# h33p/ofps

Hardware: AMD Instinct MI355X
Metric: Mvectors/s, 1080p 16x16 blocks +-16 full-search SAD (higher is better)
Workload: dtype u8

## Files before the change

### ofps_amd/csrc/sad.hip

```cpp
#include "common.hpp"

#include <cstdlib>
#include <utility>

namespace {

constexpr int kWavesPerWG = 4;

constexpr int pick_stride(int min_s, int k, int ng) {
    for (int s = min_s; s < min_s + 64; ++s)
        if ((k * s) % 32 == ng % 32) return s;
    return min_s | 1;
}

template <int B, int R, int K>
struct SadCfg {
    static_assert(B % 4 == 0 && R % 4 == 0, "tile origin must stay dword aligned");
    static_assert(B * B * 255 <= 65535, "packed u16 SAD accumulators would overflow");
    static constexpr int NCAND = 2 * R + 1;
    static constexpr int NG = (NCAND + 3) / 4;
    static constexpr int NC = (NCAND + K - 1) / K;
    static constexpr int T = NG * NC;
    static constexpr int PASSES = (T + 63) / 64;
    static constexpr int BW = B / 4;
    static constexpr int TILE_H = B + 2 * R;
    static constexpr int TILE_ROWS = NC * K + B - 1;
    static constexpr int TILE_WD = (kWavesPerWG * B + 2 * R) / 4;
    static constexpr int MAXCOL = (kWavesPerWG - 1) * BW + (NG - 1) + BW;
    static constexpr int MIN_S = (MAXCOL + 1 > TILE_WD) ? MAXCOL + 1 : TILE_WD;
    static constexpr int S = pick_stride(MIN_S, K, NG);
    static constexpr int LDS_DWORDS = TILE_ROWS * S;
};

__device__ __forceinline__ unsigned long long shfl_xor_u64(unsigned long long v, int mask) {
    unsigned lo = (unsigned)v, hi = (unsigned)(v >> 32);
    lo = __shfl_xor(lo, mask, 64);
    hi = __shfl_xor(hi, mask, 64);
    return ((unsigned long long)hi << 32) | lo;
}

struct __attribute__((packed, aligned(4))) U64A4 { unsigned long long v; };

struct SadParams {
    const uint8_t* prev_base;
    const uint8_t* cur_base;
    size_t prev_pitch, cur_pitch;
    int W, H, stride;
    int nbx, nby;
    float nx, ny;
    float4* out_entries;
    int* out_best;
    unsigned long long div_spp, div_spr;
};
inline unsigned long long div_magic48(unsigned d) { return ((1ull << 48) + d - 1) / d; }
__device__ __forceinline__ unsigned div48(unsigned n, unsigned long long m) { return (unsigned)(((unsigned long long)n * m) >> 48); }

__device__ __forceinline__ void write_block_result(const SadParams& p, int pair, int bx, int by, int B, int R,
                                                   unsigned long long key) {
    const int sad = (int)(key >> 48);
    const int dy = (int)((key >> 8) & 0xFF) - R;
    const int dx = (int)(key & 0xFF) - R;
    const size_t k = ((size_t)pair * p.nby + by) * p.nbx + bx;
    const float cx = (float)(bx * B + B / 2 + dx), cy = (float)(by * B + B / 2 + dy);
    float4 e;
    e.x = cx * p.nx;
    e.y = cy * p.ny;
    e.z = ((float)dx / 1.0f) * (-p.nx);
    e.w = ((float)dy / 1.0f) * (-p.ny);
    p.out_entries[k] = e;
    if (p.out_best) {
        p.out_best[3 * k + 0] = dx;
        p.out_best[3 * k + 1] = dy;
        p.out_best[3 * k + 2] = sad;
    }
}

template <int B, int R, int K>
__global__ __launch_bounds__(256) void sad_qsad_kernel(const SadParams p) {
    using C = SadCfg<B, R, K>;
    __shared__ uint32_t tile[C::LDS_DWORDS];

    const int pair = blockIdx.z;
    const uint8_t* __restrict__ prev = p.prev_base + (size_t)pair * p.prev_pitch;
    const uint8_t* __restrict__ cur = p.cur_base + (size_t)pair * p.cur_pitch;
    const int by = blockIdx.y;
    const int bx0 = blockIdx.x * kWavesPerWG;
    const int tid = threadIdx.x;

    const int wave = __builtin_amdgcn_readfirstlane(tid >> 6);
    const int lane = tid & 63;
    const int bx = bx0 + wave;
    const int x0 = bx * B, y0 = by * B;

    uint32_t c[B][C::BW];
    {
        const int bxc = bx < p.nbx ? bx : p.nbx - 1;
        const uint32_t* __restrict__ cp = reinterpret_cast<const uint32_t*>(cur + (size_t)y0 * p.stride + bxc * B);
        const int sdw = p.stride >> 2;
#pragma unroll
        for (int y = 0; y < B; ++y)
#pragma unroll
            for (int q = 0; q < C::BW; ++q) c[y][q] = cp[y * sdw + q];
    }

    {
        const int tx0 = bx0 * B - R, ty0 = by * B - R;
        for (int idx = tid; idx < C::TILE_H * C::TILE_WD; idx += 256) {
            const int row = idx / C::TILE_WD, col = idx - row * C::TILE_WD;
            const int gx = tx0 + 4 * col, gy = ty0 + row;
            if (gy >= 0 && gy < p.H && gx >= 0 && gx < p.W)
                tile[row * C::S + col] = *reinterpret_cast<const uint32_t*>(prev + (size_t)gy * p.stride + gx);
        }
    }
    __syncthreads();
    if (bx >= p.nbx) return;

    unsigned long long best = ~0ull;
#pragma unroll 1
    for (int pass = 0; pass < C::PASSES; ++pass) {
        const int t = pass * 64 + lane;
        const bool active = t < C::T;
        const int tc = active ? t : 0;
        const int chunk = tc / C::NG, g = tc - chunk * C::NG;
        const int dx0 = -R + 4 * g, dy0 = -R + K * chunk;

        unsigned long long acc[K];
#pragma unroll
        for (int i = 0; i < K; ++i) acc[i] = 0;

        const uint32_t* trow = tile + (K * chunk) * C::S + wave * C::BW + g;
#pragma unroll
        for (int rr = 0; rr < B + K - 1; ++rr) {
            unsigned long long win[C::BW];
#pragma unroll
            for (int q = 0; q < C::BW; ++q) win[q] = reinterpret_cast<const U64A4*>(trow + rr * C::S + q)->v;
#pragma unroll
            for (int i = 0; i < K; ++i) {
                const int y = rr - i;
                if (y >= 0 && y < B) {
#pragma unroll
                    for (int q = 0; q < C::BW; ++q) acc[i] = __builtin_amdgcn_qsad_pk_u16_u8(win[q], c[y][q], acc[i]);
                }
            }
        }
        __builtin_amdgcn_sched_group_barrier(0x100, C::BW, 0);
#pragma unroll
        for (int rr = 0; rr < B + K - 1; ++rr) {
            __builtin_amdgcn_sched_group_barrier(0x100, C::BW, 0);
            __builtin_amdgcn_sched_group_barrier(0x002, K * C::BW, 0);
        }

#pragma unroll
        for (int i = 0; i < K; ++i) asm volatile("" : "+v"(acc[i]));

        uint32_t bkey = 0xFFFFFFFFu;
        int bci = 0;
#pragma unroll
        for (int i = 0; i < K; ++i) {
            const int dy = dy0 + i;
            const int vy = (int)active & (int)(dy <= R) & (int)(y0 + dy >= 0) & (int)(y0 + dy + B <= p.H);
#pragma unroll
            for (int j = 0; j < 4; ++j) {
                const int dx = dx0 + j;
                const int v = vy & (int)(dx <= R) & (int)(x0 + dx >= 0) & (int)(x0 + dx + B <= p.W);
                const uint32_t d2inv = (uint32_t)(dx * dx + dy * dy) | (uint32_t)(v - 1);
                const uint32_t half = (j < 2) ? (uint32_t)acc[i] : (uint32_t)(acc[i] >> 32);
                const uint32_t key = ((j & 1) ? (half & 0xFFFF0000u) : (half << 16)) | d2inv;
                const bool lt = key < bkey;
                bkey = lt ? key : bkey;
                bci = lt ? (i * 4 + j) : bci;
            }
        }
        if (bkey != 0xFFFFFFFFu) {
            const int bi = bci >> 2, bj = bci & 3;
            const unsigned long long k64 =
                ((unsigned long long)bkey << 32) | (uint32_t)(((dy0 + bi + R) << 8) | (dx0 + bj + R));
            best = k64 < best ? k64 : best;
        }
    }

#pragma unroll
    for (int m = 32; m >= 1; m >>= 1) {
        const unsigned long long o = shfl_xor_u64(best, m);
        best = o < best ? o : best;
    }
    if (lane == 0) write_block_result(p, pair, bx, by, B, R, best);
}

template <int B, int R>
struct StripCfg {
    static_assert(B % 4 == 0 && R % 4 == 0, "tile origin and the dx = +R column must stay dword aligned");
    static_assert(B * B * 255 <= 65535, "packed u16 SAD accumulators would overflow");
    static constexpr int NCAND = 2 * R + 1;
    static constexpr int NGA = (2 * R) / 4;
    static constexpr int pow2_ceil(int v) { int p = 1; while (p < v) p <<= 1; return p; }
    static constexpr int NG = pow2_ceil(NGA);
    static_assert(NGA >= 1 && NG <= 64, "search range too wide for one wave per strip");
    static constexpr int NB = 64 / NG;
    static constexpr int BW = B / 4;
    static constexpr int TILE_H = B + 2 * R;
    static constexpr int KE = (NCAND + NG - 1) / NG;
    static constexpr int EDGE_COL = (2 * R) / 4;
    static constexpr int GRAN = ((NB * B) % 16 == 0 && R % 16 == 0) ? 16 : (((NB * B) % 8 == 0 && R % 8 == 0) ? 8 : 4);
    static constexpr int GDW = GRAN / 4;
    static constexpr int TILE_WG = (NB * B + 2 * R + GRAN - 1) / GRAN;
    static constexpr int MAXCOL = (NB - 1) * BW + (NG - 1) + BW;
    static constexpr int SW = ((MAXCOL + 1 > TILE_WG * GDW ? MAXCOL + 1 : TILE_WG * GDW) + 3) / 4 * 4;
    static_assert((NB - 1) * BW + EDGE_COL + BW <= SW, "edge column must lie inside a window row");
    static constexpr int TILE_ROWS = TILE_H > NG * KE + B - 1 ? TILE_H : NG * KE + B - 1;
    static constexpr int TILE_DWORDS = TILE_ROWS * SW;
    static_assert(2 * R * R < 65536, "lane key holds d2 in 16 bits");
    static constexpr int SPLIT = (NCAND + 32) / 33;
    static constexpr int NP = (NCAND + SPLIT - 1) / SPLIT;
    static constexpr int MIN_WAVES = (2 * NP + B * BW + 40 <= 168) ? 3 : 2;
    static constexpr bool COMPACT_KEY = ((2 * R * R) << 6) + NCAND < 65536 && NCAND <= 64;
    static constexpr bool RANK_KEY = !COMPACT_KEY && ((2 * R * R) << 3) + 7 < 65536;
    static constexpr int KSHIFT = COMPACT_KEY ? 6 : (RANK_KEY ? 3 : 0);
};

template <int B, int R>
struct StripWalk {
    static constexpr int ROWS_PER_BASE = (255 - StripCfg<B, R>::BW) / StripCfg<B, R>::SW + 1;
};

template <int B, int R, int I0, int RR>
__device__ __forceinline__ void strip_row(unsigned long long (&acc)[StripCfg<B, R>::NP], const uint32_t (&c)[B][B / 4],
                                          const uint32_t* lds, uint32_t& base) {
    using C = StripCfg<B, R>;
    constexpr int G = StripWalk<B, R>::ROWS_PER_BASE;
    if constexpr (RR > 0 && RR % G == 0) {
        base += G * C::SW;
        asm volatile("" : "+v"(base));
    }
    unsigned long long win[C::BW];
#pragma unroll
    for (int q = 0; q < C::BW; ++q) win[q] = reinterpret_cast<const U64A4*>(lds + base + (RR % G) * C::SW + q)->v;
#pragma unroll
    for (int ii = 0; ii < C::NP; ++ii) {
        const int y = RR - ii;
        if (I0 + ii < C::NCAND && y >= 0 && y < B) {
#pragma unroll
            for (int q = 0; q < C::BW; ++q) acc[ii] = __builtin_amdgcn_qsad_pk_u16_u8(win[q], c[y][q], acc[ii]);
        }
    }
}

template <int B, int R, int I0, int... RR>
__device__ __forceinline__ void strip_rows(unsigned long long (&acc)[StripCfg<B, R>::NP], const uint32_t (&c)[B][B / 4],
                                           const uint32_t* lds, uint32_t tile_off, std::integer_sequence<int, RR...>) {
    uint32_t base = tile_off + I0 * StripCfg<B, R>::SW;
    asm volatile("" : "+v"(base));
    (strip_row<B, R, I0, RR>(acc, c, lds, base), ...);
}

#ifndef OFPS_SAD_COLKEYS
#define OFPS_SAD_COLKEYS 2
#endif
constexpr int kSadColKeys = OFPS_SAD_COLKEYS;
constexpr int kColSlotDwords = kSadColKeys == 2 ? 4 * 64 : 0;

template <int B, int R, int I0>
__device__ __forceinline__ void strip_pass(const uint32_t (&c)[B][B / 4], const uint32_t* lds, uint32_t tile_off,
                                           const uint32_t (&colk)[4], const uint32_t (&colk_pos)[4], int y0, int H, uint32_t& bkey, int& bi,
                                           uint32_t (&colmin)[4], uint32_t* amin) {
    using C = StripCfg<B, R>;
    unsigned long long acc[C::NP];
#pragma unroll
    for (int ii = 0; ii < C::NP; ++ii) acc[ii] = 0;
    constexpr int ROWS = ((I0 + C::NP < C::NCAND ? C::NP : C::NCAND - I0) + B - 1);
    strip_rows<B, R, I0>(acc, c, lds, tile_off, std::make_integer_sequence<int, ROWS>{});
#pragma unroll
    for (int ii = 0; ii < C::NP; ++ii) asm volatile("" : "+v"(acc[ii]));
    if constexpr (kSadColKeys != 0 && (C::RANK_KEY || C::COMPACT_KEY)) {
        auto low_of = [&](int ii) -> uint32_t {
            const int i = I0 + ii, dy = -R + i;
            const bool ok = i < C::NCAND && y0 + dy >= 0 && y0 + dy + B <= H;
            return ok ? (uint32_t)(C::RANK_KEY ? ((dy * dy) << 1 | (dy > 0 ? 1 : 0)) : ((dy * dy) << 6 | i)) : 0xFFFFFFFFu;
        };
        uint32_t hmask = 0xFFFF0000u;
        asm volatile("" : "+v"(hmask));
        auto keys_of = [&](int ii, uint32_t low, uint32_t (&k)[4]) {
            const uint32_t lo = (uint32_t)acc[ii], hi = (uint32_t)(acc[ii] >> 32);
            k[0] = (lo << 16) | low; k[1] = (lo & hmask) | low; k[2] = (hi << 16) | low; k[3] = (hi & hmask) | low;
        };
        if constexpr (kSadColKeys == 1) {
#pragma unroll
            for (int ii = 0; ii < C::NP; ii += 2) {
                if (I0 + ii >= C::NCAND) break;
                uint32_t ka[4], kb[4];
                keys_of(ii, low_of(ii), ka);
                if (ii + 1 < C::NP && I0 + ii + 1 < C::NCAND) {
                    keys_of(ii + 1, low_of(ii + 1), kb);
#pragma unroll
                    for (int j = 0; j < 4; ++j)
                        asm("v_min3_u32 %0, %1, %2, %3" : "=v"(colmin[j]) : "v"(colmin[j]), "v"(ka[j]), "v"(kb[j]));
                } else {
#pragma unroll
                    for (int j = 0; j < 4; ++j) colmin[j] = min(colmin[j], ka[j]);
                }
            }
        } else {
#pragma unroll
            for (int ii = 0; ii < C::NP; ++ii) {
                if (I0 + ii >= C::NCAND) break;
                uint32_t k[4];
                keys_of(ii, low_of(ii), k);
#pragma unroll
                for (int j = 0; j < 4; ++j) __hip_atomic_fetch_min(amin + 64 * j, k[j], __ATOMIC_RELAXED, __HIP_MEMORY_SCOPE_WAVEFRONT);
            }
        }
        return;
    }
#pragma unroll
    for (int ii = 0; ii < C::NP; ++ii) {
        const int i = I0 + ii;
        const int dy = -R + i;
        if (i < C::NCAND && y0 + dy >= 0 && y0 + dy + B <= H) {
            const uint32_t lo = (uint32_t)acc[ii], hi = (uint32_t)(acc[ii] >> 32);
            const uint32_t (&ck)[4] = (C::RANK_KEY && dy > 0) ? colk_pos : colk;
            const uint32_t k0 = (lo << 16) | ck[0];
            const uint32_t k1 = (lo & 0xFFFF0000u) | ck[1];
            const uint32_t k2 = (hi << 16) | ck[2];
            const uint32_t k3 = (hi & 0xFFFF0000u) | ck[3];
            if constexpr (C::RANK_KEY) {
                bkey = min(bkey, __builtin_elementwise_add_sat(min(min(k0, k1), min(k2, k3)), (uint32_t)((dy * dy) << 3)));
            } else if constexpr (C::COMPACT_KEY) {
                const uint32_t m = __builtin_elementwise_add_sat(min(min(k0, k1), min(k2, k3)), (uint32_t)((dy * dy) << 6 | i));
                bkey = min(bkey, m);
            } else {
                const uint32_t m = __builtin_elementwise_add_sat(min(min(k0, k1), min(k2, k3)), (uint32_t)(dy * dy));
                const bool lt = m < bkey;
                bkey = lt ? m : bkey;
                bi = lt ? i : bi;
            }
        }
    }
}

template <int B, int R, int... S>
__device__ __forceinline__ void strip_passes(const uint32_t (&c)[B][B / 4], const uint32_t* lds, uint32_t tile_off,
                                             const uint32_t (&colk)[4], const uint32_t (&colk_pos)[4], int y0, int H, uint32_t& bkey, int& bi,
                                             uint32_t (&colmin)[4], uint32_t* amin, std::integer_sequence<int, S...>) {
    (strip_pass<B, R, S * StripCfg<B, R>::NP>(c, lds, tile_off, colk, colk_pos, y0, H, bkey, bi, colmin, amin), ...);
}

constexpr int kStripWaves = 4;

template <int B, int R>
__device__ __forceinline__ void strip_body(const SadParams& p, int strips_per_row, int strip, uint32_t* tiles, int wave, int lane) {
    using C = StripCfg<B, R>;
    const int strips_per_pair = strips_per_row * p.nby;
    const int pair = (int)div48((unsigned)strip, p.div_spp);
    const int rem = strip - pair * strips_per_pair;
    const int by = (int)div48((unsigned)rem, p.div_spr);
    const int bx0 = (rem - by * strips_per_row) * C::NB;

    const uint8_t* __restrict__ prev = p.prev_base + (size_t)pair * p.prev_pitch;
    const uint8_t* __restrict__ cur = p.cur_base + (size_t)pair * p.cur_pitch;
    uint32_t* tile = tiles + wave * C::TILE_DWORDS;

    const int b = lane / C::NG;
    const int g = lane % C::NG;
    const int bx = bx0 + b;
    const bool blk_on = bx < p.nbx;
    const int y0 = by * B;

    uint32_t c[B][C::BW];
    {
        const int bxc = blk_on ? bx : p.nbx - 1;
        const uint8_t* cp = cur + (size_t)y0 * p.stride + bxc * B;
#pragma unroll
        for (int y = 0; y < B; ++y) {
            if constexpr (C::BW % 4 == 0) {
#pragma unroll
                for (int q4 = 0; q4 < C::BW; q4 += 4) {
                    const uint4 v = *reinterpret_cast<const uint4*>(cp + (size_t)y * p.stride + 4 * q4);
                    c[y][q4 + 0] = v.x; c[y][q4 + 1] = v.y; c[y][q4 + 2] = v.z; c[y][q4 + 3] = v.w;
                }
            } else {
#pragma unroll
                for (int q2 = 0; q2 < C::BW; q2 += 2) {
                    const uint2 v = *reinterpret_cast<const uint2*>(cp + (size_t)y * p.stride + 4 * q2);
                    c[y][q2 + 0] = v.x; c[y][q2 + 1] = v.y;
                }
            }
        }
    }

    {
        constexpr int LR = 64 / C::TILE_WG;
        constexpr int STEPS = (C::TILE_H + LR - 1) / LR;
        const int tx0 = bx0 * B - R, ty0 = y0 - R;
        const int sr = lane / C::TILE_WG, sc = lane - sr * C::TILE_WG;
        const int gx = tx0 + C::GRAN * sc;
        const bool lane_on = sr < LR && gx >= 0 && gx < p.W;
        const uint8_t* src = prev + (ptrdiff_t)(ty0 + sr) * p.stride + gx;
        uint32_t* dst = tile + sr * C::SW + C::GDW * sc;
#pragma unroll
        for (int it = 0; it < STEPS; ++it) {
            const int row = sr + it * LR;
            const bool row_in_tile = (it + 1) * LR <= C::TILE_H || row < C::TILE_H;
            if (lane_on && row_in_tile && (unsigned)(ty0 + row) < (unsigned)p.H) {
                const uint8_t* sp = src + (ptrdiff_t)(it * LR) * p.stride;
                uint32_t* dp = dst + it * LR * C::SW;
                if constexpr (C::GRAN == 16) *reinterpret_cast<uint4*>(dp) = *reinterpret_cast<const uint4*>(sp);
                else if constexpr (C::GRAN == 8) *reinterpret_cast<uint2*>(dp) = *reinterpret_cast<const uint2*>(sp);
                else *dp = *reinterpret_cast<const uint32_t*>(sp);
            }
        }
    }
    __builtin_amdgcn_fence(__ATOMIC_RELEASE, "wavefront");
    __builtin_amdgcn_wave_barrier();
    __builtin_amdgcn_fence(__ATOMIC_ACQUIRE, "wavefront");

    const int dx0 = -R + 4 * g;
    uint32_t colk[4], colk_pos[4];
#pragma unroll
    for (int j = 0; j < 4; ++j) {
        const int dx = dx0 + j;
        const int x = bx * B + dx;
        const bool v = blk_on && g < C::NGA && x >= 0 && x + B <= p.W;
        const uint32_t rank = dx0 < 0 ? 3u - j : (uint32_t)j;
        colk[j] = v ? ((uint32_t)(dx * dx) << C::KSHIFT) | (C::RANK_KEY ? rank : 0u) : 0xFFFFFFFFu;
        colk_pos[j] = v ? ((uint32_t)(dx * dx) << C::KSHIFT) | (7u - rank) : 0xFFFFFFFFu;
    }
    uint32_t bkey = 0xFFFFFFFFu;
    int bi = 0;
    uint32_t colmin[4] = {0xFFFFFFFFu, 0xFFFFFFFFu, 0xFFFFFFFFu, 0xFFFFFFFFu};
    uint32_t* amin = nullptr;
    if constexpr (kSadColKeys == 2 && (C::RANK_KEY || C::COMPACT_KEY)) {
        amin = tiles + kStripWaves * C::TILE_DWORDS + wave * kColSlotDwords + lane;
#pragma unroll
        for (int j = 0; j < 4; ++j) amin[64 * j] = 0xFFFFFFFFu;
    }
    strip_passes<B, R>(c, tiles, (uint32_t)(wave * C::TILE_DWORDS + b * C::BW + g), colk, colk_pos, y0, p.H, bkey, bi, colmin, amin,
                       std::make_integer_sequence<int, C::SPLIT>{});
    if constexpr (kSadColKeys != 0 && (C::RANK_KEY || C::COMPACT_KEY)) {
#pragma unroll
        for (int j = 0; j < 4; ++j) {
            uint32_t kc;
            if constexpr (kSadColKeys == 2) kc = __hip_atomic_load(amin + 64 * j, __ATOMIC_RELAXED, __HIP_MEMORY_SCOPE_WAVEFRONT);
            else kc = colmin[j];
            uint32_t lk;
            if constexpr (C::RANK_KEY) {
                const uint32_t x = (((kc & 0xFFFEu) << 2) + colk[j]) ^ ((kc & 1u) * 7u);
                lk = (kc & 0xFFFF0000u) | x;
            } else {
                lk = (kc & 0xFFFF0000u) | ((kc & 0xFFFFu) + colk[j]);
            }
            lk = (colk[j] == 0xFFFFFFFFu || kc == 0xFFFFFFFFu) ? 0xFFFFFFFFu : lk;
            bkey = min(bkey, lk);
        }
    }
    unsigned long long best = ~0ull;
    if (bkey != 0xFFFFFFFFu) {
        const uint32_t d2 = (bkey & 0xFFFFu) >> C::KSHIFT;
        int dx = dx0, dy;
        if constexpr (C::RANK_KEY) {
            const int code = (int)(bkey & 7u);
            const bool neg = code < 4;
            const int rank = neg ? code : 7 - code;
            dx = dx0 + (dx0 < 0 ? 3 - rank : rank);
            const int ady = (int)(__builtin_sqrtf((float)((int)d2 - dx * dx)) + 0.5f);
            dy = neg ? -ady : ady;
        } else {
            if constexpr (C::COMPACT_KEY) bi = (int)(bkey & 63u);
            dy = -R + bi;
            const int dxsq = (int)d2 - dy * dy;
#pragma unroll
            for (int j = 1; j < 4; ++j) dx = ((dx0 + j) * (dx0 + j) == dxsq) ? dx0 + j : dx;
        }
        best = ((unsigned long long)((bkey & 0xFFFF0000u) | d2) << 32) | (unsigned long long)(uint32_t)(((dy + R) << 8) | (dx + R));
    }
    uint32_t eacc[C::KE];
#pragma unroll
    for (int i = 0; i < C::KE; ++i) eacc[i] = 0;
    {
        const uint32_t* ecol = tile + b * C::BW + C::EDGE_COL;
        const int erow0 = g * C::KE;
        uint32_t nxt[C::BW];
#pragma unroll
        for (int q = 0; q < C::BW; ++q) nxt[q] = ecol[erow0 * C::SW + q];
#pragma unroll
        for (int rr = 0; rr < B + C::KE - 1; ++rr) {
            uint32_t ref[C::BW];
#pragma unroll
            for (int q = 0; q < C::BW; ++q) ref[q] = nxt[q];
            if (rr + 1 < B + C::KE - 1) {
                const int row = erow0 + rr + 1;
#pragma unroll
                for (int q = 0; q < C::BW; ++q) nxt[q] = ecol[row * C::SW + q];
            }
#pragma unroll
            for (int i = 0; i < C::KE; ++i) {
                const int y = rr - i;
                if (y >= 0 && y < B) {
#pragma unroll
                    for (int q = 0; q < C::BW; ++q) eacc[i] = __builtin_amdgcn_sad_u8(ref[q], c[y][q], eacc[i]);
                }
            }
            asm volatile("" : "+v"(eacc[0]) : : "memory");
        }
    }

    {
        const bool xok = blk_on && bx * B + R + B <= p.W;
#pragma unroll
        for (int i = 0; i < C::KE; ++i) {
            const int dy = -R + g * C::KE + i;
            const bool v = xok && dy <= R && y0 + dy >= 0 && y0 + dy + B <= p.H;
            const unsigned long long k64 =
                ((unsigned long long)((eacc[i] << 16) | (uint32_t)(R * R + dy * dy)) << 32) |
                (unsigned long long)(uint32_t)(((dy + R) << 8) | (2 * R));
            best = (v && k64 < best) ? k64 : best;
        }
    }
#pragma unroll
    for (int m = 1; m < C::NG; m <<= 1) {
        const unsigned long long o = shfl_xor_u64(best, m);
        best = o < best ? o : best;
    }
    if (blk_on && g == 0) {
        const int sad = (int)(best >> 48);
        const int dy = (int)((best >> 8) & 0xFF) - R, dx = (int)(best & 0xFF) - R;
        const size_t k = ((size_t)pair * p.nby + by) * p.nbx + bx;
        float4 e;
        e.x = (float)(bx * B + B / 2 + dx) * p.nx;
        e.y = (float)(y0 + B / 2 + dy) * p.ny;
        e.z = ((float)dx / 1.0f) * (-p.nx);
        e.w = ((float)dy / 1.0f) * (-p.ny);
        p.out_entries[k] = e;
        if (p.out_best) {
            p.out_best[3 * k + 0] = dx;
            p.out_best[3 * k + 1] = dy;
            p.out_best[3 * k + 2] = sad;
        }
    }
}

template <int B, int R>
__global__ __launch_bounds__(64 * kStripWaves, (StripCfg<B, R>::MIN_WAVES)) void sad_strip_kernel(const SadParams p, int strips_per_row,
                                                                      int total_strips) {
    using C = StripCfg<B, R>;
    __shared__ __attribute__((aligned(16))) uint32_t tiles[kStripWaves * (C::TILE_DWORDS + kColSlotDwords)];
    const int wave = __builtin_amdgcn_readfirstlane(threadIdx.x >> 6);
    const int lane = threadIdx.x & 63;
    const int per_xcd = gridDim.x / 8;
    const int lwg = (int)(blockIdx.x % 8) * per_xcd + (int)(blockIdx.x / 8);
    const int strip = lwg * kStripWaves + wave;
    if (strip >= total_strips) return;
    strip_body<B, R>(p, strips_per_row, strip, tiles, wave, lane);
}

template <int B, int R>
__global__ __launch_bounds__(64 * kStripWaves, (StripCfg<B, R>::MIN_WAVES)) void sad_strip_list_kernel(const SadParams p, int strips_per_row,
                                                                           const uint32_t* __restrict__ strip_list) {
    using C = StripCfg<B, R>;
    __shared__ __attribute__((aligned(16))) uint32_t tiles[kStripWaves * (C::TILE_DWORDS + kColSlotDwords)];
    const int wave = __builtin_amdgcn_readfirstlane(threadIdx.x >> 6);
    const int lane = threadIdx.x & 63;
    const int count = (int)strip_list[0];
#pragma unroll 1
    for (int k = (int)blockIdx.x * kStripWaves + wave; k < count; k += (int)gridDim.x * kStripWaves)
        strip_body<B, R>(p, strips_per_row, (int)strip_list[1 + k], tiles, wave, lane);
}

struct PdeCfg {
    static constexpr int B = 16, R = 16, STEP = 4, PR = B / STEP;
    using C = StripCfg<B, R>;
    static constexpr int CUR_DW = B * C::NB * C::BW;
    static constexpr int CAP = 512;
    static constexpr int WAVE_DW = C::TILE_DWORDS + 4 + CUR_DW + CAP + 2 * C::NB;
    static constexpr int OFF_CUR = C::TILE_DWORDS + 4, OFF_LIST = OFF_CUR + CUR_DW, OFF_BEST = OFF_LIST + CAP;
    static_assert(OFF_BEST % 2 == 0, "64-bit keys must be 8-byte aligned");
};

template <int RR>
__device__ __forceinline__ void pde_row(unsigned long long (&acc)[PdeCfg::C::NP], const uint32_t (&c)[PdeCfg::PR][PdeCfg::C::BW],
                                        const uint32_t* lds, uint32_t& base) {
    using C = PdeCfg::C;
    constexpr int B = PdeCfg::B, R = PdeCfg::R, STEP = PdeCfg::STEP;
    constexpr int G = StripWalk<B, R>::ROWS_PER_BASE;
    if constexpr (RR > 0 && RR % G == 0) {
        base += G * C::SW;
        asm volatile("" : "+v"(base));
    }
    unsigned long long win[C::BW];
#pragma unroll
    for (int q = 0; q < C::BW; ++q) win[q] = reinterpret_cast<const U64A4*>(lds + base + (RR % G) * C::SW + q)->v;
#pragma unroll
    for (int ii = 0; ii < C::NP; ++ii) {
        const int y = RR - ii;
        if (ii < C::NCAND && y >= 0 && y < B && y % STEP == 0) {
#pragma unroll
            for (int q = 0; q < C::BW; ++q) acc[ii] = __builtin_amdgcn_qsad_pk_u16_u8(win[q], c[y / STEP][q], acc[ii]);
        }
    }
}
template <int... RR>
__device__ __forceinline__ void pde_rows(unsigned long long (&acc)[PdeCfg::C::NP], const uint32_t (&c)[PdeCfg::PR][PdeCfg::C::BW],
                                         const uint32_t* lds, uint32_t tile_off, std::integer_sequence<int, RR...>) {
    uint32_t base = tile_off;
    asm volatile("" : "+v"(base));
    (pde_row<RR>(acc, c, lds, base), ...);
}

__device__ __forceinline__ uint32_t pde_two_rows(const uint32_t* tile, const uint32_t* curl, int bb, int dyi, int dxi, int r8) {
    using C = PdeCfg::C;
    const int sh = dxi & 3;
    uint32_t s = 0;
#pragma unroll
    for (int k = 0; k < 2; ++k) {
        const int y = 2 * r8 + k;
        const uint32_t* rp = tile + (dyi + y) * C::SW + bb * C::BW + (dxi >> 2);
        const uint32_t* cp = curl + y * (C::NB * C::BW) + bb * C::BW;
        uint32_t d[C::BW + 1];
#pragma unroll
        for (int q = 0; q <= C::BW; ++q) d[q] = rp[q];
#pragma unroll
        for (int q = 0; q < C::BW; ++q) s = __builtin_amdgcn_sad_u8(__builtin_amdgcn_alignbyte(d[q + 1], d[q], sh), cp[q], s);
    }
    return s;
}

__global__ __launch_bounds__(64 * kStripWaves, 3) void sad_pde_kernel(const SadParams p, int strips_per_row, int total_strips,
                                                                       uint32_t* __restrict__ strip_list) {
    using P = PdeCfg;
    using C = P::C;
    constexpr int B = P::B, R = P::R;
    __shared__ __attribute__((aligned(16))) uint32_t lds[kStripWaves * P::WAVE_DW];

    const int wave = __builtin_amdgcn_readfirstlane(threadIdx.x >> 6);
    const int lane = threadIdx.x & 63;
    const int per_xcd = gridDim.x / 8;
    const int lwg = (int)(blockIdx.x % 8) * per_xcd + (int)(blockIdx.x / 8);
    const int strip = lwg * kStripWaves + wave;
    if (strip >= total_strips) return;
    const int strips_per_pair = strips_per_row * p.nby;
    const int pair = strip / strips_per_pair;
    const int rem = strip - pair * strips_per_pair;
    const int by = rem / strips_per_row;
    const int bx0 = (rem - by * strips_per_row) * C::NB;
    const uint8_t* __restrict__ prev = p.prev_base + (size_t)pair * p.prev_pitch;
    const uint8_t* __restrict__ cur = p.cur_base + (size_t)pair * p.cur_pitch;
    uint32_t* tile = lds + wave * P::WAVE_DW;
    uint32_t* curl = tile + P::OFF_CUR;
    uint32_t* list = tile + P::OFF_LIST;
    unsigned long long* bestk = reinterpret_cast<unsigned long long*>(tile + P::OFF_BEST);

    const int b = lane / C::NG, g = lane % C::NG;
    const int bx = bx0 + b;
    const bool blk_on = bx < p.nbx;
    const int y0 = by * B;

    {
        const int tx0 = bx0 * B - R, ty0 = y0 - R;
        for (int idx = lane; idx < C::TILE_H * C::TILE_WG; idx += 64) {
            const int row = idx / C::TILE_WG, col = idx - row * C::TILE_WG;
            const int gx = tx0 + 16 * col, gy = ty0 + row;
            if (gy >= 0 && gy < p.H && gx >= 0 && gx < p.W)
                *reinterpret_cast<uint4*>(tile + row * C::SW + 4 * col) = *reinterpret_cast<const uint4*>(prev + (size_t)gy * p.stride + gx);
        }
#pragma unroll
        for (int k = 0; k < 2; ++k) {
            const int idx = lane + 64 * k, row = idx / C::NB, blk = idx % C::NB;
            const int bxc = min(bx0 + blk, p.nbx - 1);
            *reinterpret_cast<uint4*>(curl + row * (C::NB * C::BW) + blk * C::BW) =
                *reinterpret_cast<const uint4*>(cur + (size_t)(y0 + row) * p.stride + bxc * B);
        }
    }
    __builtin_amdgcn_fence(__ATOMIC_RELEASE, "wavefront");
    __builtin_amdgcn_wave_barrier();
    __builtin_amdgcn_fence(__ATOMIC_ACQUIRE, "wavefront");

    uint32_t c4[P::PR][C::BW];
#pragma unroll
    for (int r = 0; r < P::PR; ++r)
#pragma unroll
        for (int q = 0; q < C::BW; ++q) c4[r][q] = curl[(P::STEP * r) * (C::NB * C::BW) + b * C::BW + q];
    unsigned long long acc[C::NP];
#pragma unroll
    for (int ii = 0; ii < C::NP; ++ii) acc[ii] = 0;
    pde_rows(acc, c4, lds, (uint32_t)(wave * P::WAVE_DW + b * C::BW + g), std::make_integer_sequence<int, C::NCAND + B - 1>{});
#pragma unroll
    for (int ii = 0; ii < C::NP; ++ii) asm volatile("" : "+v"(acc[ii]));

    const int dx0 = -R + 4 * g;
    bool colv[4];
    uint32_t colk[4];
#pragma unroll
    for (int j = 0; j < 4; ++j) {
        const int x = bx * B + dx0 + j;
        colv[j] = blk_on && x >= 0 && x + B <= p.W;
        colk[j] = colv[j] ? (uint32_t)((dx0 + j) * (dx0 + j)) << C::KSHIFT : 0xFFFFFFFFu;
    }
    static_assert(C::COMPACT_KEY && C::SPLIT == 1, "written for the +-16 geometry");
    uint32_t bkey = 0xFFFFFFFFu;
#pragma unroll
    for (int i = 0; i < C::NCAND; ++i) {
        const int dy = -R + i;
        if (y0 + dy >= 0 && y0 + dy + B <= p.H) {
            const uint32_t lo = (uint32_t)acc[i], hi = (uint32_t)(acc[i] >> 32);
            const uint32_t k0 = (lo << 16) | colk[0], k1 = (lo & 0xFFFF0000u) | colk[1];
            const uint32_t k2 = (hi << 16) | colk[2], k3 = (hi & 0xFFFF0000u) | colk[3];
            bkey = min(bkey, __builtin_elementwise_add_sat(min(min(k0, k1), min(k2, k3)), (uint32_t)((dy * dy) << 6 | i)));
        }
    }
    unsigned long long pbest = ~0ull;
    if (bkey != 0xFFFFFFFFu) {
        const int bi = (int)(bkey & 63u), dy = -R + bi;
        const uint32_t d2 = (bkey & 0xFFFFu) >> C::KSHIFT;
        const int dxsq = (int)d2 - dy * dy;
        int dx = dx0;
#pragma unroll
        for (int j = 1; j < 4; ++j) dx = ((dx0 + j) * (dx0 + j) == dxsq) ? dx0 + j : dx;
        pbest = ((unsigned long long)((bkey & 0xFFFF0000u) | d2) << 32) | (unsigned long long)(uint32_t)(((dy + R) << 8) | (dx + R));
    }
    uint32_t eacc[C::KE];
    const bool xok = blk_on && bx * B + R + B <= p.W;
    {
        const uint32_t* ecol = tile + b * C::BW + C::EDGE_COL;
#pragma unroll
        for (int i = 0; i < C::KE; ++i) {
            const int dyi = min(g * C::KE + i, C::NCAND - 1);
            uint32_t sacc = 0;
#pragma unroll
            for (int r = 0; r < P::PR; ++r)
#pragma unroll
                for (int q = 0; q < C::BW; ++q) sacc = __builtin_amdgcn_sad_u8(ecol[(dyi + P::STEP * r) * C::SW + q], c4[r][q], sacc);
            eacc[i] = sacc;
            const int dy = -R + g * C::KE + i;
            const bool v = xok && dy <= R && y0 + dy >= 0 && y0 + dy + B <= p.H;
            const unsigned long long k64 = ((unsigned long long)((sacc << 16) | (uint32_t)(R * R + dy * dy)) << 32) |
                                           (unsigned long long)(uint32_t)(((dy + R) << 8) | (2 * R));
            pbest = (v && k64 < pbest) ? k64 : pbest;
        }
    }
#pragma unroll
    for (int m = 1; m < C::NG; m <<= 1) {
        const unsigned long long o = shfl_xor_u64(pbest, m);
        pbest = o < pbest ? o : pbest;
    }
    const int dy0i = blk_on ? (int)((pbest >> 8) & 0xFF) : R, dx0i = blk_on ? (int)(pbest & 0xFF) : R;
    auto key64 = [&](uint32_t sad, int dyi, int dxi) {
        const int dy = dyi - R, dx = dxi - R;
        return ((unsigned long long)((sad << 16) | (uint32_t)(dx * dx + dy * dy)) << 32) | (unsigned long long)(uint32_t)((dyi << 8) | dxi);
    };
    uint32_t U = pde_two_rows(tile, curl, b, dy0i, dx0i, g);
#pragma unroll
    for (int m = 1; m < C::NG; m <<= 1) U += __shfl_xor(U, m, 64);
    if (g == 0) bestk[b] = blk_on ? key64(U, dy0i, dx0i) : ~0ull;
    int nlist = 0;
    {
        int uj[4];
#pragma unroll
        for (int j = 0; j < 4; ++j) uj[j] = colv[j] ? (int)U : -1;
        const unsigned long long below = (1ull << lane) - 1ull;
        typedef unsigned short us2 __attribute__((ext_vector_type(2)));
        const uint32_t u1 = min(U + 1u, 0xFFFFu) * 0x10001u;
        auto any_le = [&](uint32_t v) {
            const us2 m = __builtin_elementwise_min(__builtin_bit_cast(us2, v), __builtin_bit_cast(us2, u1));
            return __builtin_bit_cast(uint32_t, m) ^ u1;
        };
#pragma unroll
        for (int i = 0; i < C::NCAND; ++i) {
            const int dy = -R + i;
            if (y0 + dy >= 0 && y0 + dy + B <= p.H) {
                const uint32_t lo = (uint32_t)acc[i], hi = (uint32_t)(acc[i] >> 32);
                if (!__ballot((any_le(lo) | any_le(hi)) != 0u)) continue;
                const int s4[4] = {(int)(lo & 0xFFFFu), (int)(lo >> 16), (int)(hi & 0xFFFFu), (int)(hi >> 16)};
#pragma unroll
                for (int j = 0; j < 4; ++j) {
                    const bool hit = s4[j] <= uj[j];
                    const unsigned long long mask = __ballot(hit);
                    if (mask) {
                        const int pos = nlist + __popcll(mask & below);
                        if (hit && pos < P::CAP) list[pos] = ((uint32_t)b << 16) | ((uint32_t)i << 8) | (uint32_t)(4 * g + j);
                        nlist += __popcll(mask);
                    }
                }
            }
        }
#pragma unroll
        for (int i = 0; i < C::KE; ++i) {
            const int dyi = g * C::KE + i, dy = dyi - R;
            const bool hit = xok && dy <= R && y0 + dy >= 0 && y0 + dy + B <= p.H && eacc[i] <= U;
            const unsigned long long mask = __ballot(hit);
            if (mask) {
                const int pos = nlist + __popcll(mask & below);
                if (hit && pos < P::CAP) list[pos] = ((uint32_t)b << 16) | ((uint32_t)dyi << 8) | (uint32_t)(2 * R);
                nlist += __popcll(mask);
            }
        }
    }
    __builtin_amdgcn_fence(__ATOMIC_RELEASE, "wavefront");
    __builtin_amdgcn_wave_barrier();
    __builtin_amdgcn_fence(__ATOMIC_ACQUIRE, "wavefront");
    const int n = nlist;
    if (n > P::CAP) {
        if (lane == 0) {
            const uint32_t pos = atomicAdd(&strip_list[0], 1u);
            strip_list[1 + pos] = (uint32_t)strip;
        }
        return;
    }
    constexpr int PER_STEP = 2 * (64 / C::NG);
    for (int base = 0; base < n; base += PER_STEP) {
        const int idx0 = base + lane / C::NG, idx1 = idx0 + 64 / C::NG;
        const uint32_t e0 = list[min(idx0, n - 1)], e1 = list[min(idx1, n - 1)];
        const int bb0 = (int)(e0 >> 16), dyi0 = (int)((e0 >> 8) & 0xFF), dxi0 = (int)(e0 & 0xFF);
        const int bb1 = (int)(e1 >> 16), dyi1 = (int)((e1 >> 8) & 0xFF), dxi1 = (int)(e1 & 0xFF);
        uint32_t s0 = pde_two_rows(tile, curl, bb0, dyi0, dxi0, g);
        uint32_t s1 = pde_two_rows(tile, curl, bb1, dyi1, dxi1, g);
#pragma unroll
        for (int m = 1; m < C::NG; m <<= 1) { s0 += __shfl_xor(s0, m, 64); s1 += __shfl_xor(s1, m, 64); }
        if (g == 0 && idx0 < n) atomicMin(&bestk[bb0], key64(s0, dyi0, dxi0));
        if (g == 0 && idx1 < n) atomicMin(&bestk[bb1], key64(s1, dyi1, dxi1));
    }
    __builtin_amdgcn_fence(__ATOMIC_RELEASE, "wavefront");
    __builtin_amdgcn_wave_barrier();
    __builtin_amdgcn_fence(__ATOMIC_ACQUIRE, "wavefront");
    if (blk_on && g == 0) write_block_result(p, pair, bx, by, B, R, bestk[b]);
}

__global__ __launch_bounds__(64) void sad_generic_kernel(const SadParams p, int B, int R) {
    const int pair = blockIdx.z, by = blockIdx.y, bx = blockIdx.x;
    const uint8_t* __restrict__ prev = p.prev_base + (size_t)pair * p.prev_pitch;
    const uint8_t* __restrict__ cur = p.cur_base + (size_t)pair * p.cur_pitch;
    const int x0 = bx * B, y0 = by * B, n = 2 * R + 1;
    unsigned long long best = ~0ull;
    for (int cand = threadIdx.x; cand < n * n; cand += 64) {
        const int dy = cand / n - R, dx = cand % n - R;
        if (x0 + dx < 0 || x0 + dx + B > p.W || y0 + dy < 0 || y0 + dy + B > p.H) continue;
        uint32_t sad = 0;
        for (int y = 0; y < B; ++y) {
            const uint8_t* cr = cur + (size_t)(y0 + y) * p.stride + x0;
            const uint8_t* pr = prev + (size_t)(y0 + dy + y) * p.stride + x0 + dx;
            for (int x = 0; x < B; ++x) {
                const int d = (int)cr[x] - (int)pr[x];
                sad += (uint32_t)(d < 0 ? -d : d);
            }
        }
        const unsigned long long key = ((unsigned long long)sad << 32) | ((unsigned long long)(dx * dx + dy * dy) << 16) |
                                       (unsigned long long)(((dy + R) << 8) | (dx + R));
        best = key < best ? key : best;
    }
#pragma unroll
    for (int m = 32; m >= 1; m >>= 1) {
        const unsigned long long o = shfl_xor_u64(best, m);
        best = o < best ? o : best;
    }
    if (threadIdx.x == 0) {
        const int sad = (int)(best >> 32);
        const int dy = (int)((best >> 8) & 0xFF) - R, dx = (int)(best & 0xFF) - R;
        const size_t k = ((size_t)pair * p.nby + by) * p.nbx + bx;
        float4 e;
        e.x = (float)(x0 + B / 2 + dx) * p.nx;
        e.y = (float)(y0 + B / 2 + dy) * p.ny;
        e.z = ((float)dx / 1.0f) * (-p.nx);
        e.w = ((float)dy / 1.0f) * (-p.ny);
        p.out_entries[k] = e;
        if (p.out_best) {
            p.out_best[3 * k + 0] = dx;
            p.out_best[3 * k + 1] = dy;
            p.out_best[3 * k + 2] = sad;
        }
    }
}

template <int B, int R, int K>
void launch_qsad(const SadParams& p, int pairs, hipStream_t s) {
    dim3 grid((p.nbx + kWavesPerWG - 1) / kWavesPerWG, p.nby, pairs);
    hipLaunchKernelGGL((sad_qsad_kernel<B, R, K>), grid, dim3(256), 0, s, p);
}

inline void strip_div_magic(SadParams& q, int strips_per_row) {
    q.div_spp = div_magic48((unsigned)strips_per_row * (unsigned)q.nby);
    q.div_spr = div_magic48((unsigned)strips_per_row);
}

template <int B, int R>
void launch_strip(const SadParams& p, int pairs, hipStream_t s) {
    using C = StripCfg<B, R>;
    const int strips_per_row = (p.nbx + C::NB - 1) / C::NB;
    const int total = strips_per_row * p.nby * pairs;
    const int nwg = ((total + kStripWaves - 1) / kStripWaves + 7) / 8 * 8;
    SadParams q = p;
    strip_div_magic(q, strips_per_row);
    hipLaunchKernelGGL((sad_strip_kernel<B, R>), dim3(nwg), dim3(64 * kStripWaves), 0, s, q, strips_per_row, total);
}

int launch_pde_16_16(ofps_hip_ctx* ctx, const SadParams& p, int pairs, hipStream_t s) {
    using C = StripCfg<16, 16>;
    const int strips_per_row = (p.nbx + C::NB - 1) / C::NB;
    const int total = strips_per_row * p.nby * pairs;
    auto* strip_list = static_cast<uint32_t*>(ofps::scratch(ctx, ofps::S_SAD_LIST, (size_t)(total + 1) * sizeof(uint32_t)));
    if (!strip_list) return OFPS_HIP_ENOMEM;
    OFPS_HIP_TRY(ctx, hipMemsetAsync(strip_list, 0, sizeof(uint32_t), s));
    const int nwg = ((total + kStripWaves - 1) / kStripWaves + 7) / 8 * 8;
    hipLaunchKernelGGL(sad_pde_kernel, dim3(nwg), dim3(64 * kStripWaves), 0, s, p, strips_per_row, total, strip_list);
    const int nwg_ind = nwg < 8 * ctx->num_cus ? nwg : 8 * ctx->num_cus;
    SadParams q = p;
    strip_div_magic(q, strips_per_row);
    hipLaunchKernelGGL((sad_strip_list_kernel<16, 16>), dim3(nwg_ind), dim3(64 * kStripWaves), 0, s, q, strips_per_row,
                       (const uint32_t*)strip_list);
    return OFPS_HIP_OK;
}

}

extern "C" {

size_t ofps_hip_sad_block_count(int W, int H, int block) {
    if (W <= 0 || H <= 0 || block <= 0) return 0;
    return (size_t)(W / block) * (size_t)(H / block);
}

}

namespace ofps {
int sad_pairs_device(ofps_hip_ctx* ctx, const uint8_t* prev_base, size_t prev_pitch, const uint8_t* cur_base,
                     size_t cur_pitch, int pairs, int W, int H, int stride, int block, int range, void* d_out_entries,
                     void* d_out_best, bool integer_only, void* d_int_best) {
    OFPS_REQUIRE(ctx, W > 0 && H > 0 && stride >= W, "sad_flow: bad geometry W=%d H=%d stride=%d", W, H, stride);
    OFPS_REQUIRE(ctx, stride % 4 == 0 && ((uintptr_t)prev_base % 4) == 0 && ((uintptr_t)cur_base % 4) == 0 &&
                          prev_pitch % 4 == 0 && cur_pitch % 4 == 0,
                 "sad_flow: rows must be 4-byte aligned (stride=%d)", stride);
    OFPS_REQUIRE(ctx, block >= 1 && block <= 64 && range >= 0 && range <= 64,
                 "sad_flow: block=%d range=%d outside [1,64]/[0,64]", block, range);
    SadParams p{};
    p.prev_base = prev_base; p.cur_base = cur_base;
    p.prev_pitch = prev_pitch; p.cur_pitch = cur_pitch;
    p.W = W; p.H = H; p.stride = stride;
    p.nbx = W / block; p.nby = H / block;
    p.nx = 1.0f / (float)W; p.ny = 1.0f / (float)H;
    p.out_entries = static_cast<float4*>(d_out_entries);
    p.out_best = static_cast<int*>(d_out_best);
    if (p.nbx == 0 || p.nby == 0 || pairs <= 0) return OFPS_HIP_OK;
    OFPS_REQUIRE(ctx, pairs <= 65535 && p.nby <= 65535, "sad_flow: grid too large");
    OFPS_HIP_TRY(ctx, hipSetDevice(ctx->device));
    const bool qpel = ctx->opt.sad_motion_scale == 4 && !integer_only;
    if (qpel && d_int_best) p.out_best = static_cast<int*>(d_int_best);
    else if (qpel && !p.out_best) {
        p.out_best = static_cast<int*>(ofps::scratch(ctx, ofps::S_SAD_QBEST, (size_t)pairs * p.nbx * p.nby * 3 * sizeof(int)));
        if (!p.out_best) return OFPS_HIP_ENOMEM;
    }
    hipStream_t s = ctx->stream;
    const int key = block * 1000 + range;
    const bool force_block = ctx->opt.sad_force_block != 0;
    const bool strip_ok = !force_block && stride % 16 == 0 && ((uintptr_t)prev_base % 16) == 0 &&
                          ((uintptr_t)cur_base % 16) == 0 && prev_pitch % 16 == 0 && cur_pitch % 16 == 0 &&
                          (long long)p.nbx * p.nby * pairs < (1ll << 28) && (long long)p.nbx * p.nby < (1ll << 20);
    switch (key) {
        case 16016:
            if (strip_ok && ctx->sad_mode == OFPS_HIP_SAD_PRUNED) {
                const int rc = launch_pde_16_16(ctx, p, pairs, s);
                if (rc != OFPS_HIP_OK) return rc;
            } else if (strip_ok) launch_strip<16, 16>(p, pairs, s);
            else launch_qsad<16, 16, 5>(p, pairs, s);
            break;
        case 16008:
            if (strip_ok) launch_strip<16, 8>(p, pairs, s); else launch_qsad<16, 8, 3>(p, pairs, s);
            break;
        case 16032:
            if (strip_ok) launch_strip<16, 32>(p, pairs, s); else launch_qsad<16, 32, 5>(p, pairs, s);
            break;
        case 8032:
            if (strip_ok) launch_strip<8, 32>(p, pairs, s); else launch_qsad<8, 32, 5>(p, pairs, s);
            break;
        case 8016:
            if (strip_ok) launch_strip<8, 16>(p, pairs, s); else launch_qsad<8, 16, 5>(p, pairs, s);
            break;
        case 8008:
            if (strip_ok) launch_strip<8, 8>(p, pairs, s); else launch_qsad<8, 8, 3>(p, pairs, s);
            break;
#define OFPS_STRIP_CASE(BB, RR)                                         \
        case BB * 1000 + RR:                                            \
            if (strip_ok) { launch_strip<BB, RR>(p, pairs, s); break; } \
            [[fallthrough]];
        OFPS_STRIP_CASE(16, 12) OFPS_STRIP_CASE(16, 20) OFPS_STRIP_CASE(16, 24) OFPS_STRIP_CASE(16, 28)
        OFPS_STRIP_CASE(8, 12) OFPS_STRIP_CASE(8, 20) OFPS_STRIP_CASE(8, 24) OFPS_STRIP_CASE(8, 28)
#undef OFPS_STRIP_CASE
        default: {
            dim3 grid(p.nbx, p.nby, pairs);
            hipLaunchKernelGGL(sad_generic_kernel, grid, dim3(64), 0, s, p, block, range);
        }
    }
    OFPS_HIP_TRY(ctx, hipGetLastError());
    if (qpel)
        return ofps::sad_qpel_refine_device(ctx, prev_base, prev_pitch, cur_base, cur_pitch, pairs, W, H, stride, block, range, d_out_entries,
                                            p.out_best, d_out_best);
    return OFPS_HIP_OK;
}
}

extern "C" {

int ofps_hip_sad_flow_dev(ofps_hip_ctx* ctx, const void* d_frames, int n_frames, int W, int H, int stride,
                          size_t frame_pitch, int ref_mode, int block, int range, void* d_out_entries,
                          void* d_out_best) {
    if (!ctx) return OFPS_HIP_EINVAL;
    OFPS_REQUIRE(ctx, d_frames && d_out_entries, "sad_flow: null device pointer");
    OFPS_REQUIRE(ctx, n_frames >= 2, "sad_flow: need at least 2 frames (got %d)", n_frames);
    OFPS_REQUIRE(ctx, frame_pitch >= (size_t)stride * (size_t)H, "sad_flow: frame_pitch smaller than a frame");
    OFPS_REQUIRE(ctx, ref_mode == 0 || ref_mode == 1, "sad_flow: ref_mode must be 0 or 1");
    const auto* f = static_cast<const uint8_t*>(d_frames);
    return ofps::sad_pairs_device(ctx, f, ref_mode ? 0 : frame_pitch, f + frame_pitch, frame_pitch, n_frames - 1, W, H, stride,
                                  block, range, d_out_entries, d_out_best);
}

int ofps_hip_sad_flow(ofps_hip_ctx* ctx, const uint8_t* prev, const uint8_t* cur, int W, int H, int stride,
                      int block, int range, float* out_entries, int32_t* out_best, size_t* n_out) {
    if (!ctx) return OFPS_HIP_EINVAL;
    OFPS_REQUIRE(ctx, prev && cur && out_entries, "sad_flow: null host pointer");
    OFPS_REQUIRE(ctx, W > 0 && H > 0 && stride >= W && block >= 1, "sad_flow: bad geometry");
    OFPS_HIP_TRY(ctx, hipSetDevice(ctx->device));
    const int dstride = (W + 63) & ~63;
    const size_t pitch = (size_t)dstride * H;
    const size_t nblk = ofps_hip_sad_block_count(W, H, block);
    auto* d_frames = static_cast<uint8_t*>(ofps::scratch(ctx, ofps::S_FRAMES, 2 * pitch));
    auto* d_ent = static_cast<float*>(ofps::scratch(ctx, ofps::S_ENTRIES, nblk * 4 * sizeof(float)));
    auto* d_best = static_cast<int32_t*>(ofps::scratch(ctx, ofps::S_BEST, nblk * 3 * sizeof(int32_t)));
    if (!d_frames || !d_ent || !d_best) return OFPS_HIP_ENOMEM;
    OFPS_HIP_TRY(ctx, ofps::upload_rows(d_frames, dstride, prev, stride, W, H, ctx->stream));
    OFPS_HIP_TRY(ctx, ofps::upload_rows(d_frames + pitch, dstride, cur, stride, W, H, ctx->stream));
    uint32_t kept = UINT32_MAX;
    int rc;
    if (ctx->opt.sad_gate > 0 || ctx->opt.sad_consistency > 0) {
        auto* d_kept = static_cast<uint32_t*>(ofps::scratch(ctx, ofps::S_RESULT, sizeof(uint32_t)));
        if (!d_kept) return OFPS_HIP_ENOMEM;
        rc = ofps::sad_flow_filtered_device(ctx, d_frames, d_frames + pitch, W, H, dstride, block, range, ctx->opt.sad_gate, ctx->opt.sad_consistency,
                                            reinterpret_cast<float4*>(d_ent), out_best ? d_best : nullptr, d_kept);
        if (rc != OFPS_HIP_OK) return rc;
        OFPS_HIP_TRY(ctx, hipMemcpyAsync(&kept, d_kept, sizeof(kept), hipMemcpyDeviceToHost, ctx->stream));
    } else {
        rc = ofps_hip_sad_flow_dev(ctx, d_frames, 2, W, H, dstride, pitch, 0, block, range, d_ent, d_best);
        if (rc != OFPS_HIP_OK) return rc;
    }
    if (nblk) {
        OFPS_HIP_TRY(ctx, hipMemcpyAsync(out_entries, d_ent, nblk * 4 * sizeof(float), hipMemcpyDeviceToHost, ctx->stream));
        if (out_best)
            OFPS_HIP_TRY(ctx, hipMemcpyAsync(out_best, d_best, nblk * 3 * sizeof(int32_t), hipMemcpyDeviceToHost, ctx->stream));
    }
    OFPS_HIP_TRY(ctx, hipStreamSynchronize(ctx->stream));
    if (n_out) *n_out = kept < nblk ? kept : nblk;
    return OFPS_HIP_OK;
}

int ofps_hip_sad_pruned_overflow_strips(ofps_hip_ctx* ctx, uint32_t* count) {
    if (!ctx || !count) return OFPS_HIP_EINVAL;
    *count = 0;
    auto& sc = ctx->scratch[ofps::S_SAD_LIST];
    if (!sc.p) return OFPS_HIP_OK;
    OFPS_HIP_TRY(ctx, hipSetDevice(ctx->device));
    OFPS_HIP_TRY(ctx, hipStreamSynchronize(ctx->stream));
    OFPS_HIP_TRY(ctx, hipMemcpy(count, sc.p, sizeof(uint32_t), hipMemcpyDeviceToHost));
    return OFPS_HIP_OK;
}

int ofps_hip_set_sad_mode(ofps_hip_ctx* ctx, int mode) {
    if (!ctx) return OFPS_HIP_EINVAL;
    OFPS_REQUIRE(ctx, mode == OFPS_HIP_SAD_EXHAUSTIVE || mode == OFPS_HIP_SAD_PRUNED, "set_sad_mode: unknown mode %d", mode);
    ctx->sad_mode = mode;
    return OFPS_HIP_OK;
}

}
```

Before: 517.6.

## Batch unconditional clamped tile loads and overlap them with current-block loads

The reference-tile staging loop now issues every global load unconditionally, clamping addresses into the frame with v_med3, and uses a validity mask only for the LDS store. Loads are grouped into batches held in registers, and the current-block loads are placed after the last batch is issued so both sets of memory requests are in flight together. The goal is to remove per-row branching and serialised load-to-store latency in the strip prologue. In exchange it raises register pressure and adds a host-side guard that keeps 32-bit offsets from overflowing.

Result: no change. 519.8, median of 6 (+0.4%).

```diff
diff --git a/ofps_amd/csrc/sad.hip b/ofps_amd/csrc/sad.hip
--- a/ofps_amd/csrc/sad.hip
+++ b/ofps_amd/csrc/sad.hip
@@ -1,6 +1,7 @@
 #include "common.hpp"
 
 #include <cstdlib>
+#include <type_traits>
 #include <utility>
 
 namespace {
@@ -365,47 +366,69 @@
     const bool blk_on = bx < p.nbx;
     const int y0 = by * B;
 
+    constexpr int LR = 64 / C::TILE_WG;
+    constexpr int STEPS = (C::TILE_H + LR - 1) / LR;
+    constexpr int NBATCH = (STEPS + 7) / 8;
+    constexpr int BATCH = (STEPS + NBATCH - 1) / NBATCH;
+    using Gran = typename std::conditional<C::GRAN == 16, uint4, typename std::conditional<C::GRAN == 8, uint2, uint32_t>::type>::type;
     uint32_t c[B][C::BW];
     {
-        const int bxc = blk_on ? bx : p.nbx - 1;
-        const uint8_t* cp = cur + (size_t)y0 * p.stride + bxc * B;
-#pragma unroll
-        for (int y = 0; y < B; ++y) {
-            if constexpr (C::BW % 4 == 0) {
-#pragma unroll
-                for (int q4 = 0; q4 < C::BW; q4 += 4) {
-                    const uint4 v = *reinterpret_cast<const uint4*>(cp + (size_t)y * p.stride + 4 * q4);
-                    c[y][q4 + 0] = v.x; c[y][q4 + 1] = v.y; c[y][q4 + 2] = v.z; c[y][q4 + 3] = v.w;
-                }
-            } else {
-#pragma unroll
-                for (int q2 = 0; q2 < C::BW; q2 += 2) {
-                    const uint2 v = *reinterpret_cast<const uint2*>(cp + (size_t)y * p.stride + 4 * q2);
-                    c[y][q2 + 0] = v.x; c[y][q2 + 1] = v.y;
-                }
-            }
-        }
-    }
-
-    {
-        constexpr int LR = 64 / C::TILE_WG;
-        constexpr int STEPS = (C::TILE_H + LR - 1) / LR;
         const int tx0 = bx0 * B - R, ty0 = y0 - R;
         const int sr = lane / C::TILE_WG, sc = lane - sr * C::TILE_WG;
         const int gx = tx0 + C::GRAN * sc;
-        const bool lane_on = sr < LR && gx >= 0 && gx < p.W;
-        const uint8_t* src = prev + (ptrdiff_t)(ty0 + sr) * p.stride + gx;
+        const bool lane_on = sr < LR && (unsigned)gx < (unsigned)p.W;
+        int lo;
+        asm("v_med3_i32 %0, %1, 0, %2" : "=v"(lo) : "v"(gx), "s"(p.stride - C::GRAN));
+        const int hi = lo + (p.H - 1) * p.stride;
+        const int off0 = __mul24(sr, p.stride) + ty0 * p.stride + lo;
         uint32_t* dst = tile + sr * C::SW + C::GDW * sc;
 #pragma unroll
-        for (int it = 0; it < STEPS; ++it) {
-            const int row = sr + it * LR;
-            const bool row_in_tile = (it + 1) * LR <= C::TILE_H || row < C::TILE_H;
-            if (lane_on && row_in_tile && (unsigned)(ty0 + row) < (unsigned)p.H) {
-                const uint8_t* sp = src + (ptrdiff_t)(it * LR) * p.stride;
-                uint32_t* dp = dst + it * LR * C::SW;
-                if constexpr (C::GRAN == 16) *reinterpret_cast<uint4*>(dp) = *reinterpret_cast<const uint4*>(sp);
-                else if constexpr (C::GRAN == 8) *reinterpret_cast<uint2*>(dp) = *reinterpret_cast<const uint2*>(sp);
-                else *dp = *reinterpret_cast<const uint32_t*>(sp);
+        for (int bt = 0; bt < NBATCH; ++bt) {
+            Gran win[BATCH];
+            bool win_on[BATCH];
+#pragma unroll
+            for (int j = 0; j < BATCH; ++j) {
+                const int it = bt * BATCH + j;
+                if (it >= STEPS) break;
+                const int row = sr + it * LR;
+                const bool row_in_tile = (it + 1) * LR <= C::TILE_H || row < C::TILE_H;
+                const int off = off0 + it * LR * p.stride;
+                int offc;
+                asm("v_med3_i32 %0, %1, %2, %3" : "=v"(offc) : "v"(off), "v"(lo), "v"(hi));
+                win[j] = *reinterpret_cast<const Gran*>(prev + (uint32_t)offc);
+                win_on[j] = lane_on && row_in_tile && offc == off;
+            }
+            if (bt == NBATCH - 1) {
+                const int bxc = blk_on ? bx : p.nbx - 1;
+                const uint8_t* cp = cur + (size_t)y0 * p.stride + bxc * B;
+#pragma unroll
+                for (int y = 0; y < B; ++y) {
+                    if constexpr (C::BW % 4 == 0) {
+#pragma unroll
+                        for (int q4 = 0; q4 < C::BW; q4 += 4) {
+                            const uint4 v = *reinterpret_cast<const uint4*>(cp + (size_t)y * p.stride + 4 * q4);
+                            c[y][q4 + 0] = v.x; c[y][q4 + 1] = v.y; c[y][q4 + 2] = v.z; c[y][q4 + 3] = v.w;
+                        }
+                    } else {
+#pragma unroll
+                        for (int q2 = 0; q2 < C::BW; q2 += 2) {
+                            const uint2 v = *reinterpret_cast<const uint2*>(cp + (size_t)y * p.stride + 4 * q2);
+                            c[y][q2 + 0] = v.x; c[y][q2 + 1] = v.y;
+                        }
+                    }
+                }
+            }
+#pragma unroll
+            for (int j = 0; j < BATCH; ++j) {
+                if (bt * BATCH + j >= STEPS) break;
+                if constexpr (C::GRAN == 16) asm volatile("" : "+v"(win[j].x), "+v"(win[j].y), "+v"(win[j].z), "+v"(win[j].w));
+                else if constexpr (C::GRAN == 8) asm volatile("" : "+v"(win[j].x), "+v"(win[j].y));
+                else asm volatile("" : "+v"(win[j]));
+            }
+#pragma unroll
+            for (int j = 0; j < BATCH; ++j) {
+                if (bt * BATCH + j >= STEPS) break;
+                if (win_on[j]) *reinterpret_cast<Gran*>(dst + (bt * BATCH + j) * LR * C::SW) = win[j];
             }
         }
     }
@@ -950,7 +973,8 @@
     const bool force_block = ctx->opt.sad_force_block != 0;
     const bool strip_ok = !force_block && stride % 16 == 0 && ((uintptr_t)prev_base % 16) == 0 &&
                           ((uintptr_t)cur_base % 16) == 0 && prev_pitch % 16 == 0 && cur_pitch % 16 == 0 &&
-                          (long long)p.nbx * p.nby * pairs < (1ll << 28) && (long long)p.nbx * p.nby < (1ll << 20);
+                          (long long)p.nbx * p.nby * pairs < (1ll << 28) && (long long)p.nbx * p.nby < (1ll << 20) &&
+                          stride < (1 << 23) && ((long long)H + 256) * stride < (1ll << 31);
     switch (key) {
         case 16016:
             if (strip_ok && ctx->sad_mode == OFPS_HIP_SAD_PRUNED) {
```
